# X1X1010/XequiNet

Measured on AMD Instinct MI355X. Metric: edges/sec + achieved HBM GB/s, energy+force inference, QM9-shape batch, higher is better.
Workload: dtype f32

## Files before the change

include/xeq.h:

```cpp
#ifndef XEQ_H
#define XEQ_H
#include <stdint.h>

#ifdef __cplusplus
extern "C" {
#endif

enum { XEQ_F32 = 0, XEQ_F64 = 1 };
enum { XEQ_RBF_BESSEL = 0, XEQ_RBF_GAUSSIAN = 1, XEQ_RBF_EXPBERN = 2, XEQ_RBF_EXPNORM = 3 };
enum { XEQ_CUTOFF_COSINE = 0, XEQ_CUTOFF_POLYNOMIAL = 1 };
enum {
  XEQ_OK = 0,
  XEQ_ERR_INVALID_ARGUMENT = 1,
  XEQ_ERR_LAUNCH = 2,
  XEQ_ERR_UNSUPPORTED = 3
};

int xeq_version(void);
const char* xeq_last_error(void);
int64_t xeq_launch_count(void);
int64_t xeq_launch_names(int64_t first, char* buf, int64_t cap);


int xeq_csr_rowptr(const int64_t* keys, int64_t n_keys, int64_t n_rows, int32_t* rowptr, void* stream);
// ... 195 lines not shown
#define XEQ_FAMILY_WQ 0
#define XEQ_FAMILY_SB 1
#define XEQ_FAMILY_GENERIC 3
int xeq_message_auto_family(int dtype, int64_t n_nodes, int64_t n_edges, int num_basis, int node_dim, const int32_t mul[3]);
int xeq_message_wq_edges_per_stream(int64_t n_nodes, int64_t n_edges);

int xeq_edge_basis_width(int num_basis);
int xeq_message_sb_fits(int64_t n_nodes, int64_t n_edges, int num_basis, int node_dim, const int32_t mul[3]);
int xeq_edge_basis(int dtype, const void* vec, int64_t n_edges, int rbf_kind, int cutoff_kind, int num_basis,
                   double cutoff, const void* p0, const void* p1, void* basis, void* dbasis, void* stream);
int xeq_message_fwd_sb(int dtype, int64_t n_nodes, int64_t n_edges, const int32_t* rowptr, const int32_t* perm,
                       const int64_t* nbr, const void* basis, const void* h, const void* xhat, const void* s_in,
                       const void* x_in, const void* w_rbf, const void* b_rbf, int num_basis, int node_dim,
                       const int32_t mul[3], void* s_out, void* x_out, int xhat_layout, void* stream);
int xeq_message_bwd_sb(int dtype, int64_t n_nodes, int64_t n_edges, const int32_t* n_rowptr, const int32_t* n_perm,
                       const int64_t* center, const void* basis, const void* dbasis, const void* h, const void* xhat,
                       const void* grad_s, const void* grad_x, const void* w_rbf, const void* b_rbf, int num_basis,
                       int node_dim, const int32_t mul[3], void* grad_h, void* grad_xhat, void* grad_vec,
                       int xhat_layout, void* stream);

#define XEQ_SB_Y0_ZERO 8
#define XEQ_SB_ACCUM_VEC 16
#define XEQ_SB_Q_ACCUMULATE 16
#define XEQ_SB_NO_GY 32
int xeq_message_bwd_sbq(int dtype, int64_t n_nodes, int64_t n_edges, const int32_t* n_rowptr, const int32_t* n_perm,
                        const int64_t* center, const void* basis, const void* h, const void* xhat, const void* grad_s,
                        const void* grad_x, const void* w_rbf, const void* b_rbf, int num_basis, int node_dim,
                        const int32_t mul[3], void* grad_h, void* grad_xhat, void* q, void* gy, int flags, void* stream);
int xeq_message_fwd_sb_pair(int dtype, int64_t n_nodes, int64_t n_edges, const int32_t* rowptr, const int32_t* perm, const int64_t* nbr,
                            const void* basis, const void* basis_u, const void* h, const void* u_h, const void* xhat, const void* u_xhat,
                            const void* s_in, const void* x_in, const void* w_rbf, const void* b_rbf, int num_basis, int node_dim,
                            const int32_t mul[3], void* s_out, void* x_out, int xhat_layout, void* stream);
int xeq_message_bwd_sbq_pair(int dtype, int64_t n_nodes, int64_t n_edges, const int32_t* n_rowptr, const int32_t* n_perm,
                             const int64_t* center, const void* basis, const void* basis_u, const void* h, const void* u_h, const void* xhat,
                             const void* u_xhat, const void* grad_s, const void* grad_x, const void* w_rbf, const void* b_rbf, int num_basis,
                             int node_dim, const int32_t mul[3], void* grad_h, void* grad_xhat, void* q, void* gy, int flags, void* stream);
int xeq_zero_rows_from(void* buf, int64_t row_words, int64_t n_rows, const int32_t* n_valid, void* stream);
int xeq_message_q_wgrad_chunks(int64_t n_edges);
int xeq_message_q_wgrad(int dtype, const void* q, const void* basis, int64_t n_edges, int num_basis, int node_dim, const int32_t mul[3],
                        int n_chunks, void* parts, void* stream);

int xeq_message_wq_supported(int num_basis, int node_dim, const int32_t mul[3]);
int xeq_message_wq_fits(int64_t n_nodes, int64_t n_edges, int num_basis, int node_dim, const int32_t mul[3]);
int64_t xeq_message_wq_pcap(int64_t n_nodes, int64_t n_edges);
int xeq_message_wq_waves(void);
int xeq_message_wq_record_floats_for(int num_basis);
int xeq_message_wq_record_floats(void);
int64_t xeq_message_wq_plan_workspace(int64_t n_nodes);
int64_t xeq_message_wq_win_ints(int n_ranges);
int xeq_message_wq_plan(const int32_t* rowptr, const int32_t* perm, const int64_t* owner, const int64_t* gather,
                        int64_t n_nodes, int64_t n_edges, int n_ranges, void* workspace, int64_t workspace_bytes,
                        int32_t* qptr, int32_t* pgath, int32_t* peid, int32_t* qinfo, int32_t* sq, int32_t* sn, int32_t* win,
                        void* stream);
int xeq_edge_basis_wq(const void* vec, int64_t n_nodes, int64_t n_edges, const int32_t* qptr, const int32_t* peid,
                      int rbf_kind, int cutoff_kind, int num_basis, double cutoff, const void* p0, const void* p1,
                      void* basis, void* dbasis, void* stream);
int xeq_message_fwd_wq(int64_t n_nodes, int64_t n_edges, int n_ranges, const int32_t* sq, const int32_t* sn, const int32_t* win,
                       const int32_t* c_rowptr, const int32_t* pgath, const int32_t* qinfo, const void* basis, const void* h,
                       const void* xhat, const void* s_in, const void* x_in, const void* w_rbf, const void* b_rbf,
                       int num_basis, int node_dim, const int32_t mul[3], void* s_out, void* x_out, int xhat_layout,
                       void* stream);
int64_t xeq_message_wq_parts_floats(int64_t n_nodes, int64_t n_edges, const int32_t mul[3]);
#define XEQ_XHAT_HIGHER_L_ZERO 2
#define XEQ_WQ_MIRROR_WALK 4
#define XEQ_WQ_PACKED_WEIGHTS 64
int64_t xeq_message_wq_packed_weight_floats(int num_basis, int node_dim, const int32_t mul[3]);
int xeq_message_wq_pack_weights(const void* w_rbf, const void* b_rbf, int num_basis, int node_dim, const int32_t mul[3], void* packed,
                                void* stream);
int xeq_message_bwd_wq(int64_t n_nodes, int64_t n_edges, int n_ranges, const int32_t* sq, const int32_t* sn, const int32_t* win,
                       const int32_t* n_rowptr, const int32_t* pgath, const int32_t* qinfo, const void* basis,
                       const void* dbasis, const void* h, const void* xhat, const void* grad_s, const void* grad_x,
                       const void* w_rbf, const void* b_rbf, int num_basis, int node_dim, const int32_t mul[3], void* grad_h,
                       void* grad_xhat, void* parts, int xhat_layout, void* stream);
int xeq_message_wq_table_max_rows(void);
int xeq_message_wq_first_table(int family, int64_t table_rows, int training, int per_node_front);
int xeq_edge_basis_wq_table(const void* vec, int64_t n_nodes, int64_t n_edges, const int32_t* qptr, const int32_t* peid,
                            int rbf_kind, int cutoff_kind, int num_basis, double cutoff, const void* p0, const void* p1,
                            void* basis, void* dbasis, const int32_t* pgath, const int32_t* qinfo, const void* z, int z_is_int64,
                            int64_t table_rows, int32_t* slot_rows, int32_t* quad_rows, void* stream);
int xeq_message_fwd_wq_table(int64_t n_nodes, int64_t n_edges, int n_ranges, const int32_t* sq, const int32_t* sn, const int32_t* win,
                             const int32_t* c_rowptr, const int32_t* slot_rows, const int32_t* qinfo, const void* basis,
                             const void* h_table, const void* xhat0_table, int64_t table_rows, const void* s_in, const void* x_in,
                             const void* w_rbf, const void* b_rbf, int num_basis, int node_dim, const int32_t mul[3], void* s_out,
                             void* x_out, int xhat_layout, void* stream);
int xeq_message_bwd_wq_table(int64_t n_nodes, int64_t n_edges, int n_ranges, const int32_t* sq, const int32_t* sn, const int32_t* win,
                             const int32_t* n_rowptr, const int32_t* pgath, const int32_t* qinfo, const int32_t* quad_rows,
                             const void* basis, const void* dbasis, const void* h_table, const void* xhat0_table, int64_t table_rows,
                             const void* grad_s, const void* grad_x, const void* w_rbf, const void* b_rbf, int num_basis, int node_dim,
                             const int32_t mul[3], void* parts, int xhat_layout, void* stream);
int xeq_message_wq_edge_grad(const void* vec, int64_t n_nodes, int64_t n_edges, const int32_t* qptr, const int32_t* peid,
                             const int32_t* mirror, const int32_t mul[3], const void* parts, void* grad_vec, void* stream);
#define XEQ_WQ_MAX_PART_SETS 8
int xeq_message_wq_edge_grad_sum(const void* vec, int64_t n_nodes, int64_t n_edges, const int32_t* qptr, const int32_t* peid,
                                 const int32_t* mirror, const int32_t mul[3], int n_sets, const void* const* parts, void* grad_vec,
                                 void* stream);


int xeq_norm_fwd(int dtype, const void* s, const void* x, const void* ln_w, const void* ln_b, const void* eq_w,
                 const void* eq_b, int64_t n, int node_dim, const int32_t mul[3], int do_norm, void* shat, int64_t ld_s,
                 void* xhat_bt, void* stats, void* stream);
int xeq_norm_bwd(int dtype, const void* s, const void* x, const void* ln_w, const void* eq_w, const void* stats,
                 int64_t n, int node_dim, const int32_t mul[3], int do_norm, const void* g_shat, int64_t ld_gs,
                 const void* g_xhat_bt, const void* res_s, const void* res_x, void* g_s, void* g_x, void* stream);
int xeq_uv_reduce_fwd(int dtype, const void* uv_bt, int64_t n, const int32_t mul[3], double eps, void* cat,
                      int64_t ld_cat, int node_dim, void* p, void* stream);
int xeq_uv_reduce_bwd(int dtype, const void* uv_bt, const void* g_p, const void* g_cat, int64_t ld_cat, int node_dim,
// ... 135 lines not shown
```

xequinet_amd/csrc/xeq_message_wq.hip:

```cpp
#include "xeq_common.h"

#include <hipcub/hipcub.hpp>
#include <stdlib.h>

namespace xeq {

typedef float f32x16 __attribute__((ext_vector_type(16)));
typedef float f32x4 __attribute__((ext_vector_type(4)));
typedef int i32x4 __attribute__((ext_vector_type(4)));

typedef __bf16 bf16x8 __attribute__((ext_vector_type(8)));

constexpr bool wq_bftail(int ks) { return ks <= 3; }
constexpr int WQ_TAIL = 24;
constexpr int wq_tailw(int ks) { return ks <= 4 ? 4 : 8; }
constexpr int wq_recf(int ks) { return WQ_TAIL + 2 * wq_tailw(ks) + 8; }
constexpr int wq_yoff(int ks) { return WQ_TAIL + 2 * wq_tailw(ks); }
constexpr int wq_tail_values(int num_basis) { return (num_basis > 16 ? num_basis - 16 : 0) + 1; }
constexpr int wq_ks(int num_basis) {
  return wq_tail_values(num_basis) <= 1 ? 1 : (wq_tail_values(num_basis) <= 5 ? 3 : ((wq_tail_values(num_basis) + 1) / 2 < 4 ? 4 : (wq_tail_values(num_basis) + 1) / 2));
}
static_assert(wq_tailw(5) == wq_tailw(8) && wq_tailw(6) == wq_tailw(8) && wq_tailw(7) == wq_tailw(8) && !wq_bftail(5) && !wq_bftail(8),
              "records written for 5, 6 or 7 tail steps are read by the KS = 8 kernels");
constexpr int WQ_REC_MAX = 48;
static_assert(wq_recf(8) == WQ_REC_MAX && wq_recf(4) == 40 && wq_recf(1) == wq_recf(4) && wq_recf(3) == wq_recf(4), "record widths of include/xeq.h");
__device__ __forceinline__ uint32_t wq_bf16_rne(float x) {
  const uint32_t u = __float_as_uint(x);
  return (u + 0x7FFFu + ((u >> 16) & 1u)) >> 16;
}
__device__ __forceinline__ void wq_split3(float x, uint32_t& hi, uint32_t& mid, uint32_t& lo) {
  hi = wq_bf16_rne(x);
  const float r1 = x - __uint_as_float(hi << 16);
  mid = wq_bf16_rne(r1);
  const float r2 = r1 - __uint_as_float(mid << 16);
  lo = wq_bf16_rne(r2);
}
__device__ __forceinline__ int wq_tail_k(int q, int B) { return 16 + q < B ? 16 + q : (16 + q == (B > 16 ? B : 16) ? -1 : -2); }
constexpr uint32_t WQ_FIRST = 1u << 30, WQ_LAST = 1u << 31, WQ_OWNER = (1u << 30) - 1u;
#ifndef XEQ_WQ_WAVES
#define XEQ_WQ_WAVES 4
#endif
constexpr int WQ_WAVES = XEQ_WQ_WAVES;

#ifndef XEQ_WQ_PART_BWD
struct QuadCount {
  const int32_t* rowptr;
  int64_t n;
  __host__ __device__ int32_t operator()(int64_t i) const {
    if (i >= n) return 0;
    const int32_t deg = rowptr[i + 1] - rowptr[i];
    return deg > 0 ? (deg + 3) >> 2 : 1;
  }
};
#ifndef XEQ_WQ_PART_BWD
__global__ void __launch_bounds__(SCAN_WG_THREADS) k_wq_quad_scan(const QuadCount op, int32_t* __restrict__ qptr) {
  extern __shared__ int32_t scan_lds[];
  const int32_t total = wg_scan_lds(op, op.n, scan_lds);
#pragma unroll 4
  for (int64_t i = threadIdx.x; i < op.n; i += SCAN_WG_THREADS) qptr[i] = scan_lds[i];
  if (threadIdx.x == 0) qptr[op.n] = total;
}
#endif

__global__ void k_wq_fill(int64_t E, int64_t n_nodes, const int32_t* __restrict__ rowptr, const int32_t* __restrict__ perm,
                          const int64_t* __restrict__ owner, const int64_t* __restrict__ gather,
                          const int32_t* __restrict__ qptr, int32_t* __restrict__ pgath, int32_t* __restrict__ peid,
                          uint32_t* __restrict__ qinfo) {
  const int64_t s = (int64_t)blockIdx.x * blockDim.x + threadIdx.x;
  if (s >= E) {
    const int64_t n = s - E;
    if (n < n_nodes && rowptr[n] == rowptr[n + 1]) {
      const int64_t q0 = qptr[n];
      for (int i = 0; i < 4; ++i) {
        pgath[4 * q0 + i] = (int32_t)n;
        peid[4 * q0 + i] = -1;
      }
      qinfo[q0] = (uint32_t)n | WQ_FIRST | WQ_LAST;
    }
    return;
  }
  if (s >= rowptr[n_nodes]) return;
  const int32_t eid = perm ? perm[s] : (int32_t)s;
  const int64_t n = owner[eid];
  const int32_t r0 = rowptr[n], deg = rowptr[n + 1] - r0, k = (int32_t)(s - r0), q0 = qptr[n], nq = (deg + 3) >> 2;
  const int64_t p = 4 * (int64_t)q0 + k;
  pgath[p] = (int32_t)gather[eid];
  peid[p] = eid;
  if (k == deg - 1)
    for (int64_t pp = p + 1; pp < 4 * (int64_t)(q0 + nq); ++pp) {
      pgath[pp] = (int32_t)n;
      peid[pp] = -1;
    }
  if ((k & 3) == 0) {
    const int32_t g = k >> 2;
    qinfo[q0 + g] = (uint32_t)n | (g == 0 ? WQ_FIRST : 0u) | (g == nq - 1 ? WQ_LAST : 0u);
  }
}

__global__ void k_wq_streams(const int32_t* __restrict__ qptr, int64_t N, int n_ranges, int32_t* __restrict__ sq,
                             int32_t* __restrict__ sn) {
  const int k = blockIdx.x * blockDim.x + threadIdx.x;
  if (k > 2 * n_ranges) return;
  const int64_t Q = qptr[N];
  if (k == 2 * n_ranges) {
    sq[k] = (int32_t)Q;
    sn[k] = (int32_t)N;
    return;
  }
  const int64_t target = (int64_t)k * Q / (2 * n_ranges);
  int64_t lo = 0, hi = N;
  while (lo < hi) {
    const int64_t mid = (lo + hi) >> 1;
    if (qptr[mid] >= target) hi = mid;
    else lo = mid + 1;
  }
  sq[k] = qptr[lo];
  sn[k] = (int32_t)lo;
}

__global__ void k_wq_windows(const int32_t* __restrict__ sq, const int32_t* __restrict__ pgath, int n_ranges, int n_steps, int mult,
                             int32_t* __restrict__ win) {
  const int step = blockIdx.x, lane = threadIdx.x;
  if (step >= n_steps) return;
  const int k0 = min(2 * WQ_WAVES * mult * step, 2 * n_ranges), k1 = min(k0 + 2 * WQ_WAVES * mult, 2 * n_ranges);
  const int64_t p0 = 4 * (int64_t)sq[k0], p1 = 4 * (int64_t)sq[k1];
  int lo = 0x7fffffff, hi = -1;
  for (int64_t p = p0 + lane; p < p1; p += 64) {
    const int g = pgath[p];
    lo = g < lo ? g : lo;
    hi = g > hi ? g : hi;
  }
#pragma unroll
  for (int o = 32; o > 0; o >>= 1) {
    const int l2 = __shfl_xor(lo, o, 64), h2 = __shfl_xor(hi, o, 64);
    lo = l2 < lo ? l2 : lo;
    hi = h2 > hi ? h2 : hi;
  }
  if (lane == 0) {
    win[2 * step] = hi >= 0 ? lo : 0;
    win[2 * step + 1] = hi >= 0 ? hi - lo + 1 : 0;
  }
}

__device__ __forceinline__ void wq_record_piece(const float* __restrict__ vec, const int32_t* __restrict__ peid, int64_t p, int grp,
                                                const RadialSpec& rs, const float* __restrict__ p0, const float* __restrict__ p1,
                                                float* __restrict__ out, float* __restrict__ dout, int tailw, bool bftail) {
  const int yoff = WQ_TAIL + 2 * tailw;
  const int32_t e = peid[p];
  const f32x4 zero = {0.f, 0.f, 0.f, 0.f};
  if (e < 0) {
    if (grp < 2) {
#pragma unroll
      for (int c = 0; c < 3; ++c) {
        *reinterpret_cast<f32x4*>(out + 12 * grp + 4 * c) = zero;
        if (dout) *reinterpret_cast<f32x4*>(dout + 12 * grp + 4 * c) = zero;
      }
    } else if (grp < 4) {
      for (int c = 0; c < tailw; c += 4) {
        *reinterpret_cast<f32x4*>(out + WQ_TAIL + tailw * (grp - 2) + c) = zero;
        if (dout) *reinterpret_cast<f32x4*>(dout + WQ_TAIL + tailw * (grp - 2) + c) = zero;
      }
    } else {
      *reinterpret_cast<f32x4*>(out + yoff + 4 * (grp - 4)) = zero;
      if (dout) *reinterpret_cast<f32x4*>(dout + yoff + 4 * (grp - 4)) = zero;
    }
    return;
  }
  const float rc = (float)rs.cutoff;
  const EdgeGeom<float> g = edge_geom<float>(vec[3 * (int64_t)e], vec[3 * (int64_t)e + 1], vec[3 * (int64_t)e + 2]);
  const int B = rs.num_basis;
// ... 1546 lines not shown
#ifndef XEQ_WQ_PART_BWD
int xeq_message_wq_table_max_rows(void) { return WQ_TAB_MAX_ROWS; }

int xeq_message_wq_supported(int num_basis, int node_dim, const int32_t mul[3]) { return wq_supported(num_basis, node_dim, mul) ? 1 : 0; }

int xeq_message_wq_fits(int64_t n_nodes, int64_t n_edges, int num_basis, int node_dim, const int32_t mul[3]) {
  return wq_supported(num_basis, node_dim, mul) && n_nodes < (1ll << 30) && wq_fits(n_nodes, n_edges, node_dim, mul) ? 1 : 0;
}

int64_t xeq_message_wq_pcap(int64_t n_nodes, int64_t n_edges) { return wq_pcap(n_nodes, n_edges); }

int xeq_message_wq_waves(void) { return WQ_WAVES; }

int xeq_message_wq_record_floats(void) { return wq_recf(4); }
int xeq_message_wq_record_floats_for(int num_basis) { return wq_recf(wq_ks(num_basis)); }

int64_t xeq_message_wq_plan_workspace(int64_t n_nodes) {
  size_t temp = 0;
  QuadCount op{nullptr, n_nodes};
  hipcub::CountingInputIterator<int64_t> cnt(0);
  hipcub::TransformInputIterator<int32_t, QuadCount, hipcub::CountingInputIterator<int64_t>> it(cnt, op);
  if (hipcub::DeviceScan::ExclusiveSum(nullptr, temp, it, (int32_t*)nullptr, (int)(n_nodes + 1)) != hipSuccess) return -1;
  return (int64_t)temp + 256;
}

int xeq_message_wq_plan(const int32_t* rowptr, const int32_t* perm, const int64_t* owner, const int64_t* gather,
                        int64_t n_nodes, int64_t n_edges, int n_ranges, void* workspace, int64_t workspace_bytes,
                        int32_t* qptr, int32_t* pgath, int32_t* peid, int32_t* qinfo, int32_t* sq, int32_t* sn, int32_t* win,
                        void* stream) {
  XEQ_CHECK_ARG(n_nodes >= 0 && n_edges >= 0 && n_ranges >= 1 && n_nodes < (1ll << 30) && n_edges < (1ll << 31), "xeq_message_wq_plan: bad sizes");
  const int64_t need = xeq_message_wq_plan_workspace(n_nodes);
  XEQ_CHECK_ARG(need >= 0 && workspace_bytes >= need, "xeq_message_wq_plan: workspace of %lld bytes, need %lld", (long long)workspace_bytes, (long long)need);
  QuadCount op{rowptr, n_nodes};
  if (n_nodes <= SCAN_WG_MAX_ITEMS) {
    static const bool attr_ok = hipFuncSetAttribute((const void*)k_wq_quad_scan, hipFuncAttributeMaxDynamicSharedMemorySize,
                                                    (int)wg_scan_lds_bytes(SCAN_WG_MAX_ITEMS)) == hipSuccess;
    XEQ_CHECK_ARG(attr_ok, "xeq_message_wq_plan: cannot reserve LDS for the quad scan");
    hipLaunchKernelGGL(k_wq_quad_scan, dim3(1), dim3(SCAN_WG_THREADS), wg_scan_lds_bytes(n_nodes), (hipStream_t)stream, op, qptr);
    XEQ_CHECK_LAUNCH("xeq_message_wq_plan (quad scan)");
  } else {
    hipcub::CountingInputIterator<int64_t> cnt(0);
    hipcub::TransformInputIterator<int32_t, QuadCount, hipcub::CountingInputIterator<int64_t>> it(cnt, op);
    size_t temp = (size_t)workspace_bytes;
    if (hipcub::DeviceScan::ExclusiveSum(workspace, temp, it, qptr, (int)(n_nodes + 1), (hipStream_t)stream) != hipSuccess) {
      xeq::set_error("xeq_message_wq_plan: scan failed");
      return XEQ_ERR_LAUNCH;
    }
  }
  if (n_edges + n_nodes > 0) {
    hipLaunchKernelGGL(k_wq_fill, dim3((unsigned)((n_edges + n_nodes + 255) / 256)), dim3(256), 0, (hipStream_t)stream, n_edges, n_nodes,
                       rowptr, perm, owner, gather, (const int32_t*)qptr, pgath, peid, (uint32_t*)qinfo);
    XEQ_CHECK_LAUNCH("xeq_message_wq_plan (fill)");
  }
  const int n = 2 * n_ranges + 1;
  hipLaunchKernelGGL(k_wq_streams, dim3((unsigned)((n + 255) / 256)), dim3(256), 0, (hipStream_t)stream, (const int32_t*)qptr,
                     n_nodes, n_ranges, sq, sn);
  XEQ_CHECK_LAUNCH("xeq_message_wq_plan (streams)");
  const int n_steps = wq_class_steps(n_ranges, 1);
  hipLaunchKernelGGL(k_wq_windows, dim3((unsigned)n_steps), dim3(64), 0, (hipStream_t)stream, (const int32_t*)sq,
                     (const int32_t*)pgath, n_ranges, n_steps, 1, win);
  XEQ_CHECK_LAUNCH("xeq_message_wq_plan (windows)");
  const int mlong = wq_long_mult(n_edges, n_ranges);
  if (mlong > 1) {
    const int n_long = wq_class_steps(n_ranges, mlong);
    hipLaunchKernelGGL(k_wq_windows, dim3((unsigned)n_long), dim3(64), 0, (hipStream_t)stream, (const int32_t*)sq,
                       (const int32_t*)pgath, n_ranges, n_long, mlong, win + 2 * n_steps);
    XEQ_CHECK_LAUNCH("xeq_message_wq_plan (windows, long class)");
  }
  return XEQ_OK;
}

int64_t xeq_message_wq_win_ints(int n_ranges) {
  return 2 * ((int64_t)wq_class_steps(n_ranges, 1) + (int64_t)wq_class_steps(n_ranges, 2) + 1);
}

static int wq_edge_basis(const void* vec, int64_t n_nodes, int64_t n_edges, const int32_t* qptr, const int32_t* peid,
                         int rbf_kind, int cutoff_kind, int num_basis, double cutoff, const void* p0, const void* p1,
                         void* basis, void* dbasis, const WqTableIndex& ti, void* stream) {
  XEQ_CHECK_ARG(n_edges >= 0 && n_nodes >= 0 && num_basis >= 1 && num_basis <= 31 && cutoff > 0, "xeq_edge_basis_wq: bad sizes");
  XEQ_CHECK_ARG(rbf_kind >= XEQ_RBF_BESSEL && rbf_kind <= XEQ_RBF_EXPNORM, "xeq_edge_basis_wq: rbf kernel %d is not implemented", rbf_kind);
  XEQ_CHECK_ARG(rbf_kind == XEQ_RBF_BESSEL || p1 != nullptr, "xeq_edge_basis_wq: this radial basis needs its second parameter array (std / logc / mu)");
  XEQ_CHECK_ARG(cutoff_kind == XEQ_CUTOFF_COSINE || cutoff_kind == XEQ_CUTOFF_POLYNOMIAL, "xeq_edge_basis_wq: cutoff function %d is not implemented", cutoff_kind);
  if (n_edges == 0 && n_nodes == 0) return XEQ_OK;
  const int64_t pcap = wq_pcap(n_nodes, n_edges), total = (pcap + WQ_REC_SLOTS - 1) / WQ_REC_SLOTS * 256;
  const int ks = wq_ks(num_basis);
  XEQ_CHECK_ARG(pcap * wq_recf(ks) < (1ll << 31) * 2, "xeq_edge_basis_wq: too many edges for 32-bit record offsets (shard the batch)");
  RadialSpec rs{rbf_kind, cutoff_kind, num_basis, cutoff};
  hipLaunchKernelGGL(k_wq_records, dim3((unsigned)((total + 255) / 256)), dim3(256), 0, (hipStream_t)stream, (const float*)vec,
                     peid, qptr, n_nodes, pcap, rs, (const float*)p0, (const float*)p1, (float*)basis, (float*)dbasis, wq_recf(ks), wq_tailw(ks), wq_bftail(ks) ? 1 : 0, ti);
  XEQ_CHECK_LAUNCH("xeq_edge_basis_wq");
  return XEQ_OK;
}
int xeq_edge_basis_wq(const void* vec, int64_t n_nodes, int64_t n_edges, const int32_t* qptr, const int32_t* peid,
                      int rbf_kind, int cutoff_kind, int num_basis, double cutoff, const void* p0, const void* p1,
                      void* basis, void* dbasis, void* stream) {
  return wq_edge_basis(vec, n_nodes, n_edges, qptr, peid, rbf_kind, cutoff_kind, num_basis, cutoff, p0, p1, basis, dbasis, WqTableIndex{}, stream);
}
int xeq_edge_basis_wq_table(const void* vec, int64_t n_nodes, int64_t n_edges, const int32_t* qptr, const int32_t* peid,
                            int rbf_kind, int cutoff_kind, int num_basis, double cutoff, const void* p0, const void* p1,
                            void* basis, void* dbasis, const int32_t* pgath, const int32_t* qinfo, const void* z, int z_is_int64,
                            int64_t table_rows, int32_t* slot_rows, int32_t* quad_rows, void* stream) {
  XEQ_CHECK_ARG(pgath && qinfo && z && slot_rows && quad_rows && table_rows >= 1, "xeq_edge_basis_wq_table: NULL argument / empty table");
  const WqTableIndex ti{z, z_is_int64, table_rows, pgath, (const uint32_t*)qinfo, slot_rows, quad_rows};
  return wq_edge_basis(vec, n_nodes, n_edges, qptr, peid, rbf_kind, cutoff_kind, num_basis, cutoff, p0, p1, basis, dbasis, ti, stream);
}

static int wq_ks_template(int num_basis) {
  const int ks = wq_ks(num_basis);
  return ks <= 1 ? 1 : (ks <= 3 ? 3 : (ks <= 4 ? 4 : 8));
}
int64_t xeq_message_wq_packed_weight_floats(int num_basis, int node_dim, const int32_t mul[3]) {
  if (!wq_supported(num_basis, node_dim, mul)) return -1;
  const int kst = wq_ks_template(num_basis);
  const int64_t per_unit = 3 * (int64_t)(3 * 64 * 4 + (wq_bftail(kst) ? 3 * 64 * 4 : kst * 64));
  return per_unit * (mul[0] / 32 + mul[1] / 32 + mul[2] / 32);
}
int xeq_message_wq_pack_weights(const void* w_rbf, const void* b_rbf, int num_basis, int node_dim, const int32_t mul[3], void* packed,
                                void* stream) {
  WqArgs a{};
  int rcode = wq_check("xeq_message_wq_pack_weights", 0, 0, 1, num_basis, node_dim, mul, a);
  if (rcode != XEQ_OK) return rcode;
// ... 185 lines not shown
```

xequinet_amd/lib.py:

```python
from __future__ import annotations

import ctypes
import os
from ctypes import c_char_p, c_double, c_int, c_int32, c_int64, c_uint64, c_void_p
from typing import Optional

import torch

_HERE = os.path.dirname(os.path.abspath(__file__))
LIB_PATH = os.environ.get("XEQ_LIB_PATH") or os.path.join(_HERE, "libxeq_hip.so")

XEQ_F32, XEQ_F64 = 0, 1
COPY_MANY_MAX = 16
MD_CHUNK = 256
SB_ACCUM_VEC = 16
XHAT_HIGHER_L_ZERO = 2
SB_Y0_ZERO = 8
SB_Q_ACCUMULATE = 16
SB_NO_GY = 32
WQ_MIRROR_WALK = 4
WQ_PACKED_WEIGHTS = 64
WQ_MAX_PART_SETS = 8
RBF_KINDS = {"bessel": 0, "gaussian": 1, "expbern": 2, "expnorm": 3}
CUTOFF_KINDS = {"cosine": 0, "polynomial": 1}
# ... 61 lines not shown
    "xeq_copy_many": [c_int, ctypes.POINTER(c_void_p), ctypes.POINTER(c_void_p), ctypes.POINTER(c_int64), _P],
    "xeq_compare_many": [c_int, ctypes.POINTER(c_void_p), ctypes.POINTER(c_void_p), ctypes.POINTER(c_int64), ctypes.c_int32, _P, _P],
    "xeq_tensor_product_path": [c_int, _P, _P, c_int64, c_int, c_int, c_int, c_int, c_int, c_int, c_int, c_int, c_int, c_int, c_int,
                                c_int, c_int, _P, _P, c_int64, c_double, _P, _P],
    "xeq_tensor_product": [c_int, _P, _P, c_int64, c_int, c_int, c_int, c_int, ctypes.POINTER(ctypes.c_int32), _P, ctypes.POINTER(ctypes.c_int32),
                           c_int, _P, c_int64, ctypes.POINTER(ctypes.c_int32), ctypes.POINTER(c_double), _P, _P],
    "xeq_tensor_product_wgrad": [c_int, _P, _P, _P, c_int64, c_int, c_int, c_int, c_int, ctypes.POINTER(ctypes.c_int32), _P,
                                 ctypes.POINTER(ctypes.c_int32), ctypes.POINTER(ctypes.c_int32), ctypes.POINTER(ctypes.c_int32), c_int,
                                 ctypes.POINTER(c_double), c_int, _P, _P],
    "xeq_tensor_product_wgrad_chunks": [c_int64],
    "xeq_scatter_add": [c_int, _P, _P, c_int64, c_int64, _P, c_int64, _P],
    "xeq_message_fwd": [c_int, c_int64, c_int64, _P, _P, _P, _P, _P, _P, _P, _P, _P, _P, _P, _P,
                        c_int, c_int, c_int, c_double, c_int, _I3, _P, _P, c_int, _P],
    "xeq_message_bwd": [c_int, c_int64, c_int64, _P, _P, _P, _P, _P, _P, _P, _P, _P, _P, _P, _P,
                        c_int, c_int, c_int, c_double, c_int, _I3, _P, _P, _P, c_int, _P],
    "xeq_message_param_grad_parts": [c_int64],
    "xeq_message_param_grad": [c_int, c_int64, c_int64, _P, _P, _P, _P, _P, _P, _P, _P, _P, _P, c_int, c_int, c_int, c_double, c_int,
                               _I3, c_int, c_int, _P, _P],
    "xeq_message_param_grad_mc_supported": [c_int, c_int, c_int, c_int, _I3],
    "xeq_param_basis_width": [c_int, c_int],
    "xeq_message_param_grad_mc_parts": [c_int64, c_int, _I3],
    "xeq_param_basis": [_P, c_int64, c_int, c_int, c_int, c_double, _P, _P, _P, _P],
    "xeq_message_param_grad_mc": [c_int64, c_int64, _P, _P, _P, _P, _P, _P, _P, c_int, c_int, c_int, _I3, c_int, c_int, _P, c_int, _P, _P],
    "xeq_to_bt": [_P, c_int64, _I3, _P, _P],
    "xeq_norm_param_grad_chunks": [c_int64],
    "xeq_norm_param_grad": [_P, _P, _P, _P, c_int64, _P, c_int64, c_int, _I3, c_int, _P, _P],
    "xeq_message_auto_family": [c_int, c_int64, c_int64, c_int, c_int, _I3],
    "xeq_message_wq_edges_per_stream": [c_int64, c_int64],
    "xeq_edge_basis_width": [c_int],
    "xeq_edge_basis": [c_int, _P, c_int64, c_int, c_int, c_int, c_double, _P, _P, _P, _P, _P],
    "xeq_message_fwd_sb": [c_int, c_int64, c_int64, _P, _P, _P, _P, _P, _P, _P, _P, _P, _P, c_int, c_int, _I3, _P, _P, c_int, _P],
    "xeq_message_bwd_sbq": [c_int, c_int64, c_int64, _P, _P, _P, _P, _P, _P, _P, _P, _P, _P, c_int, c_int, _I3, _P, _P, _P, _P, c_int, _P],
    "xeq_message_q_wgrad": [c_int, _P, _P, c_int64, c_int, c_int, _I3, c_int, _P, _P],
    "xeq_message_q_wgrad_chunks": [c_int64],
    "xeq_train_norm": [c_int, c_int, c_int64, _P, _P, _P, _P, _P, _P, _P, _P, _P, _P, c_int, _I3, c_double, c_double, c_int, _P, _P, _P, _P],
    "xeq_train_uv": [c_int, c_int, c_int64, _P, _P, _P, _I3, c_double, _P, _P, _P],
    "xeq_train_out": [c_int, c_int, c_int64, _P, _P, _P, _P, _P, _P, _P, _P, c_int, _I3, _P, _P, _P, _P],
    "xeq_train_edge_supported": [c_int, c_int, c_int, c_int],
    "xeq_train_edge": [c_int, c_int, c_int64, _P, _P, _P, _P, c_int, c_int, c_int, c_double, _P, _P, _P, _P],
    "xeq_zero_rows_from": [_P, c_int64, c_int64, _P, _P],
    "xeq_message_fwd_sb_pair": [c_int, c_int64, c_int64, _P, _P, _P, _P, _P, _P, _P, _P, _P, _P, _P, _P, _P, c_int, c_int, _I3, _P, _P, c_int, _P],
    "xeq_message_bwd_sbq_pair": [c_int, c_int64, c_int64, _P, _P, _P, _P, _P, _P, _P, _P, _P, _P, _P, _P, _P, c_int, c_int, _I3, _P, _P, _P, _P, c_int, _P],
    "xeq_message_bwd_sb": [c_int, c_int64, c_int64, _P, _P, _P, _P, _P, _P, _P, _P, _P, _P, _P, c_int, c_int, _I3, _P, _P, _P,
                           c_int, _P],
    "xeq_message_sb_fits": [c_int64, c_int64, c_int, c_int, _I3],
    "xeq_message_wq_supported": [c_int, c_int, _I3],
    "xeq_message_wq_fits": [c_int64, c_int64, c_int, c_int, _I3],
    "xeq_message_wq_pcap": [c_int64, c_int64],
    "xeq_message_wq_waves": [],
    "xeq_message_wq_record_floats": [],
    "xeq_message_wq_record_floats_for": [c_int],
    "xeq_message_wq_plan_workspace": [c_int64],
    "xeq_message_wq_win_ints": [c_int],
    "xeq_message_wq_plan": [_P, _P, _P, _P, c_int64, c_int64, c_int, _P, c_int64, _P, _P, _P, _P, _P, _P, _P, _P],
    "xeq_edge_basis_wq": [_P, c_int64, c_int64, _P, _P, c_int, c_int, c_int, c_double, _P, _P, _P, _P, _P],
    "xeq_message_fwd_wq": [c_int64, c_int64, c_int, _P, _P, _P, _P, _P, _P, _P, _P, _P, _P, _P, _P, _P, c_int, c_int, _I3,
                           _P, _P, c_int, _P],
    "xeq_message_wq_table_max_rows": [],
    "xeq_message_wq_first_table": [c_int, c_int64, c_int, c_int],
    "xeq_edge_basis_wq_table": [_P, c_int64, c_int64, _P, _P, c_int, c_int, c_int, c_double, _P, _P, _P, _P, _P, _P, _P, c_int, c_int64, _P, _P, _P],
    "xeq_message_fwd_wq_table": [c_int64, c_int64, c_int, _P, _P, _P, _P, _P, _P, _P, _P, _P, c_int64, _P, _P, _P, _P, c_int, c_int, _I3,
                                 _P, _P, c_int, _P],
    "xeq_message_bwd_wq_table": [c_int64, c_int64, c_int, _P, _P, _P, _P, _P, _P, _P, _P, _P, _P, _P, c_int64, _P, _P, _P, _P, c_int, c_int,
                                 _I3, _P, c_int, _P],
    "xeq_message_wq_parts_floats": [c_int64, c_int64, _I3],
    "xeq_message_bwd_wq": [c_int64, c_int64, c_int, _P, _P, _P, _P, _P, _P, _P, _P, _P, _P, _P, _P, _P, _P, c_int, c_int,
                           _I3, _P, _P, _P, c_int, _P],
    "xeq_message_wq_packed_weight_floats": [c_int, c_int, _I3],
    "xeq_message_wq_pack_weights": [_P, _P, c_int, c_int, _I3, _P, _P],
    "xeq_message_wq_edge_grad": [_P, c_int64, c_int64, _P, _P, _P, _I3, _P, _P, _P],
    "xeq_message_wq_edge_grad_sum": [_P, c_int64, c_int64, _P, _P, _P, _I3, c_int, ctypes.POINTER(c_void_p), _P, _P],
    "xeq_norm_fwd": [c_int, _P, _P, _P, _P, _P, _P, c_int64, c_int, _I3, c_int, _P, c_int64, _P, _P, _P],
    "xeq_norm_bwd": [c_int, _P, _P, _P, _P, _P, c_int64, c_int, _I3, c_int, _P, c_int64, _P, _P, _P, _P, _P, _P],
    "xeq_uv_reduce_fwd": [c_int, _P, c_int64, _I3, c_double, _P, c_int64, c_int, _P, _P],
    "xeq_uv_reduce_bwd": [c_int, _P, _P, _P, c_int64, c_int, c_int64, _I3, c_double, _P, _P, _P, _P],
    "xeq_update_out_fwd": [c_int, _P, _P, _P, _P, _P, c_int64, c_int, _I3, _P, _P, _P],
    "xeq_update_out_bwd": [c_int, _P, _P, _P, _P, _P, c_int64, c_int, _I3, _P, _P, _P, _P],
    "xeq_update_uv_supported": [c_int, c_int, _I3],
    "xeq_update_uv_fwd": [_P, _P, _P, _P, _P, _P, c_int64, c_int, _I3, c_int, _P, _P, _P, c_int, c_double, _P, c_int64, _P, _P, _P, _P],
    "xeq_update_uv_bwd": [_P, _P, _P, c_int64, _P, _P, _P, c_int64, _P, _P, _P, _P, _P, c_int64, c_int, _I3, c_int, _P, _P, _P, c_double,
                          _P, _P, _P, _P],
    "xeq_mlp2_supported": [c_int, c_int, c_int, c_int],
    "xeq_node_tile_split": [c_int64, c_int, ctypes.POINTER(c_int64)],
    "xeq_mlp_packed_floats": [c_int, c_int],
    "xeq_mlp_pack": [_P, _P, c_int, c_int, c_int, _P, _P],
    "xeq_mlp2_fwd": [_P, c_int64, c_int64, c_int, _P, _P, c_int, _P, _P, c_int64, _P],
    "xeq_mlp2_bwd": [_P, c_int64, c_int64, c_int, _P, _P, _P, c_int, _P, c_int64, _P],
    "xeq_mlp2h_supported": [c_int, c_int, c_int, c_int],
    "xeq_mlp2h_fwd": [c_int, _P, c_int64, c_int64, c_int, c_int, _P, _P, c_int, _P, _P, c_int64, _P],
    "xeq_mlp2h_bwd": [c_int, _P, c_int64, c_int64, c_int, c_int, _P, _P, _P, c_int, _P, c_int64, _P],
    "xeq_mlp2_and_linear": [c_int, _P, c_int64, c_int64, c_int, _P, _P, c_int, _P, _P, c_int64, _P, c_int64, c_int, _P, c_int, _P, c_int64, _P],
    "xeq_pack_epoch": [],
    "xeq_pack_epoch_bump": [],
    "xeq_rowptr_guard": [_P, c_int64, c_int64, _P, _P, _P],
    "xeq_node_block_supported": [c_int, c_int, _I3],
    "xeq_node_block_fwd_tiles": [c_int],
    "xeq_node_block_rows": [c_int64],
    "xeq_node_block_auto": [c_int64],
    "xeq_small_rows_limit": [],
    "xeq_node_block_set_waves": [c_int],
    "xeq_node_block_pack_fwd": [_P, _P, _P, _P, _P, _P, _P, _P, _P, _P],
    "xeq_node_block_fwd": [c_int64, _P, _P, _P, _P, _P, _P, _P, _P, _P, c_double, _P, _P, _P, _P, _P, _P, _P, _P, _P, _P, _P, _P, _P, _P, _P,
                           _P, _P, _P, _P, _P],
    "xeq_node_block_linear_test": [_P, c_int64, _P, c_int, c_int, _P, _P, _P],
    "xeq_node_block_bwd_tiles": [c_int, c_int],
    "xeq_node_block_pack_bwd": [_P, _P, _P, _P, _P, _P, _P, _P, c_int, _P, _P],
# ... 143 lines not shown
```

Before: 185.7 million.

## Split wave-quad streams by tile-balanced greedy walks instead of equal quad counts

```diff
diff --git a/include/xeq.h b/include/xeq.h
--- a/include/xeq.h
+++ b/include/xeq.h
@@ -271,6 +271,7 @@
                         int64_t n_nodes, int64_t n_edges, int n_ranges, void* workspace, int64_t workspace_bytes,
                         int32_t* qptr, int32_t* pgath, int32_t* peid, int32_t* qinfo, int32_t* sq, int32_t* sn, int32_t* win,
                         void* stream);
+int xeq_message_wq_stream_table(const int32_t* qptr, int64_t n_nodes, int n_ranges, int32_t* sq, int32_t* sn);
 int xeq_edge_basis_wq(const void* vec, int64_t n_nodes, int64_t n_edges, const int32_t* qptr, const int32_t* peid,
                       int rbf_kind, int cutoff_kind, int num_basis, double cutoff, const void* p0, const void* p1,
                       void* basis, void* dbasis, void* stream);
diff --git a/xequinet_amd/csrc/xeq_message_wq.hip b/xequinet_amd/csrc/xeq_message_wq.hip
--- a/xequinet_amd/csrc/xeq_message_wq.hip
+++ b/xequinet_amd/csrc/xeq_message_wq.hip
@@ -2,6 +2,7 @@
 
 #include <hipcub/hipcub.hpp>
 #include <stdlib.h>
+#include <string.h>
 
 namespace xeq {
 
@@ -97,25 +98,220 @@
   }
 }
 
-__global__ void k_wq_streams(const int32_t* __restrict__ qptr, int64_t N, int n_ranges, int32_t* __restrict__ sq,
-                             int32_t* __restrict__ sn) {
-  const int k = blockIdx.x * blockDim.x + threadIdx.x;
-  if (k > 2 * n_ranges) return;
-  const int64_t Q = qptr[N];
-  if (k == 2 * n_ranges) {
-    sq[k] = (int32_t)Q;
-    sn[k] = (int32_t)N;
-    return;
-  }
-  const int64_t target = (int64_t)k * Q / (2 * n_ranges);
-  int64_t lo = 0, hi = N;
+constexpr int WQ_SBLOCK = 64;
+constexpr int WQ_SBLOCK_NODES = 4096;
+struct WqStreamDims {
+  int64_t Q;
+  int S, T0, n_blocks;
+};
+__host__ __device__ inline WqStreamDims wq_stream_dims(int64_t Q, int n_ranges) {
+  WqStreamDims d;
+  d.Q = Q;
+  d.S = 2 * n_ranges;
+  const int64_t t0 = (Q + 2 * (int64_t)d.S) / (4 * (int64_t)d.S);
+  d.T0 = t0 < 1 ? 1 : (int)t0;
+  d.n_blocks = (d.S + WQ_SBLOCK - 1) / WQ_SBLOCK;
+  return d;
+}
+__host__ __device__ inline void wq_block_nodes(const int32_t* __restrict__ qptr, int64_t N, const WqStreamDims& d, int b, int64_t& n0,
+                                               int64_t& n1) {
+  const int64_t t0 = (int64_t)b * WQ_SBLOCK * d.Q / d.S, t1 = (int64_t)(b + 1) * WQ_SBLOCK * d.Q / d.S;
+  int64_t lo0 = 0, hi0 = N, lo1 = 0, hi1 = N;
+  while (lo0 < hi0 || lo1 < hi1) {
+    const int64_t m0 = (lo0 + hi0) >> 1, m1 = (lo1 + hi1) >> 1;
+    const int32_t v0 = qptr[m0], v1 = qptr[m1];
+    if (lo0 < hi0) {
+      if (v0 >= t0) hi0 = m0;
+      else lo0 = m0 + 1;
+    }
+    if (lo1 < hi1) {
+      if (v1 >= t1) hi1 = m1;
+      else lo1 = m1 + 1;
+    }
+  }
+  n0 = lo0;
+  n1 = b + 1 >= d.n_blocks ? N : lo1;
+}
+struct WqWalk {
+  int tiles;
+  int fits;
+};
+template <class QF, class NextF, class StoreF>
+__host__ __device__ inline WqWalk wq_walk_block(QF q, NextF next, int64_t n0, int64_t n1, int nb, int T, StoreF store) {
+  WqWalk w = {0, 1};
+  int64_t n = n0, qn = q(n0);
+  int prev = 0;
+  for (int j = 0; j < nb; ++j) {
+    int64_t e = n, qe = qn;
+    if (n < n1) {
+      if (j == nb - 1) {
+        e = n1;
+        qe = q(n1);
+      } else {
+        e = next(n, qn + 4 * (int64_t)T, qe);
+        if (e == n) {
+          e = n + 1;
+          qe = q(e);
+        }
+      }
+    }
+    const int len = (int)(qe - qn);
+    if (j == nb - 1 && len > 4 * T && e - n > 1) w.fits = 0;
+    if (j & 1) w.tiles += ((prev > len ? prev : len) + 3) >> 2;
+    else prev = len;
+    store(j, e);
+    n = e;
+    qn = qe;
+  }
+  if (nb & 1) w.tiles += (prev + 3) >> 2;
+  return w;
+}
+constexpr int WQ_WALKS = 4;
+__host__ __device__ inline int wq_pick_walk(const int tiles[WQ_WALKS], const int fits[WQ_WALKS], int tiles_equal) {
+  int best = -1;
+  for (int v = 0; v < WQ_WALKS - 1; ++v)
+    if (tiles[v] >= 0 && fits[v] && (best < 0 || tiles[v] < tiles[best])) best = v;
+  if (best < 0 && fits[WQ_WALKS - 1]) best = WQ_WALKS - 1;
+  return best < 0 || tiles[best] > tiles_equal ? WQ_WALKS : best;
+}
+template <class QF>
+__host__ __device__ inline int64_t wq_equal_first(QF q, int64_t n0, int64_t n1, const WqStreamDims& d, int64_t k) {
+  const int64_t target = k * d.Q / d.S;
+  int64_t lo = n0, hi = n1;
   while (lo < hi) {
     const int64_t mid = (lo + hi) >> 1;
-    if (qptr[mid] >= target) hi = mid;
+    if ((int64_t)q(mid) >= target) hi = mid;
     else lo = mid + 1;
   }
-  sq[k] = qptr[lo];
-  sn[k] = (int32_t)lo;
+  return lo;
+}
+template <class QF>
+__host__ __device__ inline int wq_equal_range(QF q, int64_t n0, int64_t n1, const WqStreamDims& d, int b, int r, int nb, int64_t& e0, int64_t& e1) {
+  const int64_t k = (int64_t)b * WQ_SBLOCK + 2 * r;
+  const int64_t f = r == 0 ? n0 : wq_equal_first(q, n0, n1, d, k);
+  e0 = wq_equal_first(q, n0, n1, d, k + 1);
+  e1 = 2 * r + 2 >= nb ? n1 : wq_equal_first(q, n0, n1, d, k + 2);
+  const int l0 = (int)(q(e0) - q(f)), l1 = (int)(q(e1) - q(e0));
+  return ((l0 > l1 ? l0 : l1) + 3) >> 2;
+}
+enum { WQ_RULE_TILES = 0, WQ_RULE_EQUAL = 1 };
+static int wq_stream_rule() {
+  const char* env = getenv("XEQ_WQ_STREAM_RULE");
+  return env && strcmp(env, "equal") == 0 ? WQ_RULE_EQUAL : WQ_RULE_TILES;
+}
+
+__global__ void __launch_bounds__(64 * (WQ_WALKS + 1)) k_wq_streams(const int32_t* __restrict__ qptr, int64_t N, int n_ranges, int rule,
+                                                    int32_t* __restrict__ sq, int32_t* __restrict__ sn) {
+  const int64_t Q = qptr[N];
+  if (rule == WQ_RULE_EQUAL) {
+    const int k = blockIdx.x * blockDim.x + threadIdx.x;
+    if (k > 2 * n_ranges) return;
+    if (k == 2 * n_ranges) {
+      sq[k] = (int32_t)Q;
+      sn[k] = (int32_t)N;
+      return;
+    }
+    const int64_t target = (int64_t)k * Q / (2 * n_ranges);
+    int64_t lo = 0, hi = N;
+    while (lo < hi) {
+      const int64_t mid = (lo + hi) >> 1;
+      if (qptr[mid] >= target) hi = mid;
+      else lo = mid + 1;
+    }
+    sq[k] = qptr[lo];
+    sn[k] = (int32_t)lo;
+    return;
+  }
+  __shared__ int32_t qs[WQ_SBLOCK_NODES];
+  __shared__ int32_t ends[WQ_WALKS + 1][WQ_SBLOCK];
+  __shared__ int res_tiles[WQ_WALKS + 1], res_fits[WQ_WALKS];
+  const int b = blockIdx.x, wave = __builtin_amdgcn_readfirstlane((int)(threadIdx.x >> 6)), lane = threadIdx.x & 63;
+  const WqStreamDims d = wq_stream_dims(Q, n_ranges);
+  if (b >= d.n_blocks || wave > WQ_WALKS) return;
+  auto first_at_or_behind = [&](int64_t target) -> int64_t {
+    int lo = 0, hi = (int)N;
+    while (lo < hi) {
+      const int step = (hi - lo + 63) >> 6, m = lo + lane * step;
+      const int c = __popcll(__ballot(m < hi && (int64_t)qptr[m] < target));
+      if (c == 0) hi = lo;
+      else {
+        hi = lo + c * step < hi ? lo + c * step : hi;
+        lo = lo + (c - 1) * step + 1;
+      }
+    }
+    return lo;
+  };
+  const int64_t n0 = first_at_or_behind((int64_t)b * WQ_SBLOCK * d.Q / d.S);
+  const int64_t n1 = b + 1 >= d.n_blocks ? N : first_at_or_behind((int64_t)(b + 1) * WQ_SBLOCK * d.Q / d.S);
+  const int cnt = (int)(n1 - n0);
+  const bool in_lds = cnt < WQ_SBLOCK_NODES;
+  if (in_lds)
+    for (int i = threadIdx.x; i <= cnt; i += blockDim.x) qs[i] = qptr[n0 + i];
+  __syncthreads();
+  const int nb = d.S - b * WQ_SBLOCK < WQ_SBLOCK ? d.S - b * WQ_SBLOCK : WQ_SBLOCK;
+  auto candidates = [&](auto q, auto next) {
+    if (wave < WQ_WALKS) {
+      const int T = d.T0 - 1 + wave;
+      WqWalk w = {-1, 0};
+      if (T >= 1) w = wq_walk_block(q, next, n0, n1, nb, T, [&](int j, int64_t e) {
+        if (lane == 0) ends[wave][j] = (int32_t)e;
+      });
+      if (lane == 0) {
+        res_tiles[wave] = w.tiles;
+        res_fits[wave] = w.fits;
+      }
+    } else {
+      int t = 0;
+      if (2 * lane < nb) {
+        int64_t e0, e1;
+        t = wq_equal_range(q, n0, n1, d, b, lane, nb, e0, e1);
+        ends[WQ_WALKS][2 * lane] = (int32_t)e0;
+        ends[WQ_WALKS][2 * lane + 1] = (int32_t)e1;
+      }
+#pragma unroll
+      for (int o = 32; o > 0; o >>= 1) t += __shfl_xor(t, o, 64);
+      if (lane == 0) res_tiles[WQ_WALKS] = t;
+    }
+  };
+  if (in_lds) {
+    candidates([&](int64_t n) -> int32_t { return qs[(int)(n - n0)]; },
+               [&](int64_t n, int64_t limit, int64_t& qe) -> int64_t {
+                 int e = (int)(n - n0);
+                 for (;;) {
+                   const int m = e + 1 + lane;
+                   const int v = m <= cnt ? qs[m] : 0x7fffffff;
+                   const int c = __popcll(__ballot((int64_t)v <= limit));
+                   if (c > 0) qe = __builtin_amdgcn_readlane(v, c - 1);
+                   e += c;
+                   if (c < 64) return n0 + e;
+                 }
+               });
+  } else {
+    candidates([&](int64_t n) -> int32_t { return qptr[n]; },
+               [&](int64_t n, int64_t limit, int64_t& qe) -> int64_t {
+                 int64_t e = n;
+                 for (;;) {
+                   const int64_t m = e + 1 + lane;
+                   const int v = m <= n1 ? qptr[m] : 0x7fffffff;
+                   const int c = __popcll(__ballot((int64_t)v <= limit));
+                   if (c > 0) qe = __builtin_amdgcn_readlane(v, c - 1);
+                   e += c;
+                   if (c < 64) return e;
+                 }
+               });
+  }
+  __syncthreads();
+  const int pick = wq_pick_walk(res_tiles, res_fits, res_tiles[WQ_WALKS]);
+  const int j = threadIdx.x;
+  if (j < nb) {
+    const int64_t first = j == 0 ? n0 : (int64_t)ends[pick][j - 1];
+    sq[b * WQ_SBLOCK + j] = in_lds ? qs[(int)(first - n0)] : qptr[first];
+    sn[b * WQ_SBLOCK + j] = (int32_t)first;
+  }
+  if (b == d.n_blocks - 1 && threadIdx.x == 0) {
+    sq[d.S] = (int32_t)Q;
+    sn[d.S] = (int32_t)N;
+  }
 }
 
 __global__ void k_wq_windows(const int32_t* __restrict__ sq, const int32_t* __restrict__ pgath, int n_ranges, int n_steps, int mult,
@@ -1768,9 +1964,14 @@
                        rowptr, perm, owner, gather, (const int32_t*)qptr, pgath, peid, (uint32_t*)qinfo);
     XEQ_CHECK_LAUNCH("xeq_message_wq_plan (fill)");
   }
-  const int n = 2 * n_ranges + 1;
-  hipLaunchKernelGGL(k_wq_streams, dim3((unsigned)((n + 255) / 256)), dim3(256), 0, (hipStream_t)stream, (const int32_t*)qptr,
-                     n_nodes, n_ranges, sq, sn);
+  if (wq_stream_rule() == WQ_RULE_EQUAL) {
+    const int n = 2 * n_ranges + 1;
+    hipLaunchKernelGGL(k_wq_streams, dim3((unsigned)((n + 255) / 256)), dim3(256), 0, (hipStream_t)stream, (const int32_t*)qptr,
+                       n_nodes, n_ranges, (int)WQ_RULE_EQUAL, sq, sn);
+  } else {
+    hipLaunchKernelGGL(k_wq_streams, dim3((unsigned)((2 * n_ranges + WQ_SBLOCK - 1) / WQ_SBLOCK)), dim3(64 * (WQ_WALKS + 1)), 0, (hipStream_t)stream,
+                       (const int32_t*)qptr, n_nodes, n_ranges, (int)WQ_RULE_TILES, sq, sn);
+  }
   XEQ_CHECK_LAUNCH("xeq_message_wq_plan (streams)");
   const int n_steps = wq_class_steps(n_ranges, 1);
   hipLaunchKernelGGL(k_wq_windows, dim3((unsigned)n_steps), dim3(64), 0, (hipStream_t)stream, (const int32_t*)sq,
@@ -1783,6 +1984,49 @@
                        (const int32_t*)pgath, n_ranges, n_long, mlong, win + 2 * n_steps);
     XEQ_CHECK_LAUNCH("xeq_message_wq_plan (windows, long class)");
   }
+  return XEQ_OK;
+}
+
+int xeq_message_wq_stream_table(const int32_t* qptr, int64_t n_nodes, int n_ranges, int32_t* sq, int32_t* sn) {
+  XEQ_CHECK_ARG(qptr != nullptr && sq != nullptr && sn != nullptr && n_nodes >= 0 && n_nodes < (1ll << 30) && n_ranges >= 1 &&
+                    n_ranges < (1 << 29),
+                "xeq_message_wq_stream_table: bad arguments");
+  const WqStreamDims d = wq_stream_dims(qptr[n_nodes], n_ranges);
+  for (int b = 0; b < d.n_blocks; ++b) {
+    int64_t n0, n1;
+    wq_block_nodes(qptr, n_nodes, d, b, n0, n1);
+    const int nb = d.S - b * WQ_SBLOCK < WQ_SBLOCK ? d.S - b * WQ_SBLOCK : WQ_SBLOCK;
+    auto q = [&](int64_t n) -> int32_t { return qptr[n]; };
+    auto next = [&](int64_t n, int64_t limit, int64_t& qe) -> int64_t {
+      int64_t e = n;
+      while (e < n1 && (int64_t)qptr[e + 1] <= limit) ++e;
+      if (e > n) qe = qptr[e];
+      return e;
+    };
+    int32_t ends[WQ_WALKS + 1][WQ_SBLOCK];
+    int tiles[WQ_WALKS], fits[WQ_WALKS], tiles_equal = 0;
+    for (int r = 0; 2 * r < nb; ++r) {
+      int64_t e0, e1;
+      tiles_equal += wq_equal_range(q, n0, n1, d, b, r, nb, e0, e1);
+      ends[WQ_WALKS][2 * r] = (int32_t)e0;
+      ends[WQ_WALKS][2 * r + 1] = (int32_t)e1;
+    }
+    for (int v = 0; v < WQ_WALKS; ++v) {
+      const int T = d.T0 - 1 + v;
+      WqWalk w = {-1, 0};
+      if (T >= 1) w = wq_walk_block(q, next, n0, n1, nb, T, [&](int j, int64_t e) { ends[v][j] = (int32_t)e; });
+      tiles[v] = w.tiles;
+      fits[v] = w.fits;
+    }
+    const int pick = wq_pick_walk(tiles, fits, tiles_equal);
+    for (int j = 0; j < nb; ++j) {
+      const int64_t first = j == 0 ? n0 : (int64_t)ends[pick][j - 1];
+      sq[b * WQ_SBLOCK + j] = qptr[first];
+      sn[b * WQ_SBLOCK + j] = (int32_t)first;
+    }
+  }
+  sq[d.S] = (int32_t)d.Q;
+  sn[d.S] = (int32_t)n_nodes;
   return XEQ_OK;
 }
 
diff --git a/xequinet_amd/lib.py b/xequinet_amd/lib.py
--- a/xequinet_amd/lib.py
+++ b/xequinet_amd/lib.py
@@ -137,6 +137,7 @@
     "xeq_message_wq_record_floats_for": [c_int],
     "xeq_message_wq_plan_workspace": [c_int64],
     "xeq_message_wq_win_ints": [c_int],
+    "xeq_message_wq_stream_table": [_P, c_int64, c_int, _P, _P],
     "xeq_message_wq_plan": [_P, _P, _P, _P, c_int64, c_int64, c_int, _P, c_int64, _P, _P, _P, _P, _P, _P, _P, _P],
     "xeq_edge_basis_wq": [_P, c_int64, c_int64, _P, _P, c_int, c_int, c_int, c_double, _P, _P, _P, _P, _P],
     "xeq_message_fwd_wq": [c_int64, c_int64, c_int, _P, _P, _P, _P, _P, _P, _P, _P, _P, _P, _P, _P, _P, c_int, c_int, _I3,
```

After: 183.6 million (median of 2 runs). No clear change (-1.1%).
